# LPMP/BDD

Hardware: AMD Instinct MI355X
Metric: parallel-MMA iterations/sec, 10.5M BDD nodes, 1 GPU (+ achieved HBM GB/s in roofline) (higher is better)
Workload: dtype f32

## Files before the change

bdd_amd/capi.py:

```python
from __future__ import annotations

import ctypes as C
import os
import subprocess

_HERE = os.path.dirname(os.path.abspath(__file__))
LIB_PATH = os.path.abspath(os.environ["BDDMMA_LIB"]) if os.environ.get("BDDMMA_LIB") else os.path.join(_HERE, "csrc", "libbdd_mma_hip.so")

OK = 0
ERR_INVALID_ARGUMENT, ERR_INVALID_BDD, ERR_DEVICE, ERR_STATE, ERR_UNSUPPORTED, ERR_IO = -1, -2, -3, -4, -5, -6
F32, F64 = 0, 1
K_FORWARD_MM, K_BACKWARD_MM, K_FINISH_DELTA, K_OTHER, K_COUNT = 0, 1, 2, 3, 4


class Options(C.Structure):
    _fields_ = [("pack_width", C.c_uint32), ("wide_pack_width", C.c_uint32), ("deterministic", C.c_uint32),
                ("vars_per_bin", C.c_uint32), ("stage_cap", C.c_uint32), ("waves_per_block", C.c_uint32),
                ("keep_bdd_order", C.c_uint32), ("resident_sweeps", C.c_uint32), ("exchange_by_variable", C.c_uint32),
                ("variant_flags", C.c_uint32), ("pack_fill", C.c_uint32), ("pack_stagger", C.c_uint32)]


class LbfgsParams(C.Structure):
    _fields_ = [("history_size", C.c_int32), ("init_step_size", C.c_double), ("req_rel_lb_increase", C.c_double),
                ("step_size_decrease_factor", C.c_double), ("step_size_increase_factor", C.c_double)]
# ... 26 lines not shown
    "bddmma_nr_variables": (_U64, [_V]),
    "bddmma_nr_bdds": (_U64, [_V]),
    "bddmma_nr_layers": (_U64, [_V]),
    "bddmma_nr_bdd_nodes": (_U64, [_V]),
    "bddmma_nr_hops": (_U64, [_V]),
    "bddmma_nr_packs": (_U64, [_V]),
    "bddmma_solve_sweep_kind": (_I, [_V]),
    "bddmma_fused_small": (_I, [_V]),
    "bddmma_fused_small_learned": (_I, [_V]),
    "bddmma_fused_small_history": (_I, [_V]),
    "bddmma_fused_small_stop": (_I, [_V]),
    "bddmma_nontemporal_loads": (_I, [_V]),
    "bddmma_potentials_on_chip": (_I, [_V]),
    "bddmma_onchip_hops": (_I, [_V]),
    "bddmma_lane_sweeps": (_I, [_V]),
    "bddmma_precision": (_I, [_V]),
    "bddmma_device": (_I, [_V]),
    "bddmma_num_bdds_per_var": (_I, [_V, _V]),
    "bddmma_layer_variables": (_I, [_V, _V]),
    "bddmma_layer_bdds": (_I, [_V, _V]),
    "bddmma_nodes_per_hop": (_I, [_V, _V]),
    "bddmma_layers_per_hop": (_I, [_V, _V]),
    "bddmma_update_costs": (_I, [_V, _V, _U64, _V, _U64, _I, _I]),
    "bddmma_set_cost": (_I, [_V, _D, _U64]),
    "bddmma_get_solver_costs": (_I, [_V, _V, _V, _V, _I]),
    "bddmma_set_solver_costs": (_I, [_V, _V, _V, _V, _I]),
    "bddmma_primal_objective_vec": (_I, [_V, _V, _I]),
    "bddmma_forward_run": (_I, [_V]),
    "bddmma_backward_run": (_I, [_V]),
    "bddmma_lower_bound": (_I, [_V, C.POINTER(_D)]),
# ... 71 lines not shown
    "bddmma_set_profiling": (_I, [_V, _I]),
    "bddmma_get_profile": (_I, [_V, C.POINTER(Profile)]),
    "bddmma_time_iterations": (_I, [_V, _D, _U64, C.POINTER(_D)]),
    "bddmma_time_kernel": (_I, [_V, _I, _U64, C.POINTER(_D)]),
    "bddmma_device_bytes": (_U64, [_V]),
    "bddmma_device_allocated_bytes": (_U64, [_V]),
    "bddmma_layout_create": (_I, [C.POINTER(_V), _V, _V, _U64, C.POINTER(Options)]),
    "bddmma_layout_create_for_chip": (_I, [C.POINTER(_V), _V, _V, _U64, C.POINTER(Options), _I, C.c_uint32, C.c_uint32]),
    "bddmma_layout_destroy": (None, [_V]),
    "bddmma_layout_size": (_U64, [_V, _I]),
    "bddmma_layout_copy": (_I, [_V, _I, _V]),
    "bddmma_layout_res2_records": (_I, [_V, _I, _V, _V, _V]),
    "bddmma_layout_stream_records": (_I, [_V, _I, _V, _V, _V]),
    "bddmma_layout_layer_records": (_I, [_V, _I, _V, _V, _V]),
    "bddmma_layout_lane_codes": (_I, [_V, _I, _V, _V, _V]),
    "bddmma_layout_seg_exchange": (_I, [_V, _I, _I, _V, _V, _V, _V]),
}

_I64P, _U64P = C.POINTER(C.c_int64), C.POINTER(C.c_uint64)
ILP_SIGNATURES = {
    "bddilp_last_error": (C.c_char_p, []),
    "bddilp_parse_lp": (_I, [C.c_char_p, C.POINTER(_V)]),
    "bddilp_parse_opb": (_I, [C.c_char_p, C.POINTER(_V)]),
    "bddilp_parse": (_I, [C.c_char_p, C.POINTER(_V)]),
    "bddilp_destroy": (None, [_V]),
    "bddilp_nr_variables": (_U64, [_V]),
    "bddilp_nr_constraints": (_U64, [_V]),
    "bddilp_variable_name": (C.c_char_p, [_V, _U64]),
    "bddilp_objective": (_I, [_V, _V, C.POINTER(_D)]),
    "bddilp_constraint_size": (_U64, [_V, _U64]),
# ... 53 lines not shown
```

bdd_amd/csrc/capi.cpp:

```cpp
#include <chrono>
#include <cmath>
#include <cstdio>
#include <cstdlib>
#include <cstring>
#include <limits>
#include <new>
#include <string>
#include <vector>

#include "../../include/bdd_mma.h"
#include "layout.hpp"
#include "solver.hpp"

using namespace bddmma;

struct bddmma_lbfgs;
extern "C" int bddmma_lbfgs_iteration(bddmma_lbfgs* l);
extern "C" int bddmma_lbfgs_update_costs(bddmma_lbfgs* l, const void* lo, uint64_t n_lo, const void* hi, uint64_t n_hi, int elem_precision,
                                         int on_device);

namespace {
thread_local std::string g_err;

template <typename F>
// ... 122 lines not shown
uint64_t bddmma_nr_variables(const bddmma_solver* s) { return s && s->impl ? s->impl->n_vars : 0; }
uint64_t bddmma_nr_bdds(const bddmma_solver* s) { return s && s->impl ? s->impl->n_bdds : 0; }
uint64_t bddmma_nr_layers(const bddmma_solver* s) { return s && s->impl ? s->impl->n_layers : 0; }
uint64_t bddmma_nr_bdd_nodes(const bddmma_solver* s) { return s && s->impl ? s->impl->n_input_nodes : 0; }
uint64_t bddmma_nr_hops(const bddmma_solver* s) { return s && s->impl ? s->impl->n_hops : 0; }
uint64_t bddmma_nr_packs(const bddmma_solver* s) { return s && s->impl ? s->impl->n_packs_narrow + s->impl->n_packs_wide : 0; }
int bddmma_solve_sweep_kind(const bddmma_solver* s) { return s && s->impl ? s->impl->solve_sweep_kind : -1; }
int bddmma_fused_small(const bddmma_solver* s) { return s && s->impl ? (s->impl->fused_small ? 1 : 0) : -1; }
int bddmma_fused_small_learned(const bddmma_solver* s) { return s && s->impl ? (s->impl->fused_small_learned ? 1 : 0) : -1; }
int bddmma_fused_small_history(const bddmma_solver* s) { return s && s->impl ? (s->impl->fused_small_history ? 1 : 0) : -1; }
int bddmma_fused_small_stop(const bddmma_solver* s) { return s && s->impl ? (s->impl->fused_small_stop ? 1 : 0) : -1; }
int bddmma_nontemporal_loads(const bddmma_solver* s) { return s && s->impl ? (s->impl->nt_loads ? 1 : 0) : -1; }
int bddmma_potentials_on_chip(const bddmma_solver* s) { return s && s->impl ? (s->impl->pot_on_chip ? 1 : 0) : -1; }
int bddmma_onchip_hops(const bddmma_solver* s) { return s && s->impl ? s->impl->onchip_hops : -1; }
int bddmma_lane_sweeps(const bddmma_solver* s) { return s && s->impl ? (s->impl->lane_sweeps ? 1 : 0) : -1; }
int bddmma_precision(const bddmma_solver* s) { return s && s->impl ? s->impl->precision : -1; }
int bddmma_device(const bddmma_solver* s) { return s && s->impl ? s->impl->device : -1; }
uint64_t bddmma_device_bytes(const bddmma_solver* s) { return s && s->impl ? s->impl->dev_bytes : 0; }
uint64_t bddmma_device_allocated_bytes(const bddmma_solver* s) { return s && s->impl ? s->impl->dev_alloc_bytes : 0; }

int bddmma_num_bdds_per_var(const bddmma_solver* s, int32_t* out)
{
    return guarded(s, [&](SolverBase* b) { return copy_host(b->h_nbdds, out); });
}
int bddmma_layer_variables(const bddmma_solver* s, int32_t* out)
{
    return guarded(s, [&](SolverBase* b) { return copy_host(b->h_layer_var, out); });
}
int bddmma_layer_bdds(const bddmma_solver* s, int32_t* out)
{
// ... 799 lines not shown
}

int bddmma_layout_lane_codes(const bddmma_layout* l, int real_size, uint32_t* info, uint32_t* words, uint32_t* code_off)
{
    if (!l || !info || (real_size != 4 && real_size != 8)) return BDDMMA_ERR_INVALID_ARGUMENT;
    LayerRecords R;
    build_layer_records(l->L, (uint32_t)real_size, R);
    LaneCodes K;
    build_lane_codes(l->L, (uint32_t)real_size, R, K);
    info[0] = K.ok ? 1u : 0u; info[1] = (uint32_t)K.words.size(); info[2] = K.affine ? 1u : 0u;
    if (words && !K.words.empty()) std::memcpy(words, K.words.data(), K.words.size() * sizeof(uint32_t));
    if (code_off && !K.code_off.empty()) std::memcpy(code_off, K.code_off.data(), K.code_off.size() * sizeof(uint32_t));
    return BDDMMA_OK;
}

}
```

bdd_amd/csrc/kernels/narrow5.hpp:

```cpp
#pragma once

namespace bddmma {

#ifndef BDDMMA_N5_WAVES
#define BDDMMA_N5_WAVES 5
#endif
constexpr int n5_waves(int hc) { return hc <= 10 ? BDDMMA_N5_WAVES : 4; }

__device__ __forceinline__ uint32_t lane_hop_code(const u4v& cw, int h) { return (cw[h / 3] >> (10 * (h % 3))) & 0x3FFu; }
__device__ __forceinline__ u4v lane_codes_again(const u4v& cw)
{
    uint32_t a = cw[0], b = cw[1], c = cw[2], e = cw[3];
    asm volatile("" : "+v"(a), "+v"(b), "+v"(c), "+v"(e));
    return u4v{a, b, c, e};
}
__device__ __forceinline__ uint32_t lane_bit(uint32_t code, uint32_t bit) { return (uint32_t)__builtin_amdgcn_sbfe((int)code, bit, 1u); }
__device__ __forceinline__ float lane_pick(uint32_t m, float a, float b)
{
    return __builtin_bit_cast(float, (m & __builtin_bit_cast(uint32_t, a)) | (~m & __builtin_bit_cast(uint32_t, b)));
}
__device__ __forceinline__ float lane_child(uint32_t code, uint32_t k, float ta, float tb)
{
    const uint32_t odd = lane_bit(code, k), snk = lane_bit(code, k + 1);
    const float node = lane_pick(odd, tb, ta);
// ... 1 lines not shown
    return lane_pick(snk, sink, node);
}
__device__ __forceinline__ void lane_push(float& fa, float& fb, uint32_t code, float p0, float p1, float p2, float p3)
{
    const float INF = inf_v<float>();
    const float pv[4] = {p0, p1, p2, p3};
    fa = fb = INF;
#pragma unroll
    for (uint32_t k = 0; k < 4; ++k) {
        const uint32_t odd = lane_bit(code, 2 * k), snk = lane_bit(code, 2 * k + 1);
        fa = rmin(fa, lane_pick(odd | snk, INF, pv[k]));
        fb = rmin(fb, lane_pick(odd & ~snk, pv[k], INF));
    }
}

template <typename REAL, int WPB, int HC>
__device__ __forceinline__ void fwd_narrow5_body(const DevPtrs<REAL>& d, const PackDev& pk, const uint32_t* __restrict__ lcode,
                                                 const uint32_t* __restrict__ lcode_off, uint32_t lcode_words, REAL omega, uint32_t block_id)
{
    static_assert(HC + 1 <= (int)HOP_WIN, "one window of hop offsets has to hold the pack");
    static_assert(HC <= (int)LCODE_HOPS, "a lane's code words hold LCODE_HOPS hops");
    using P2 = typename Pair<REAL>::type;
    extern __shared__ __attribute__((aligned(16))) unsigned char dyn_lds[];
    P2* sD = reinterpret_cast<P2*>(dyn_lds);
    __shared__ uint32_t sOffN_[WPB][HOP_WIN], sOffL_[WPB][HOP_WIN], sOffR_[WPB][HOP_WIN];
    const uint32_t tid = threadIdx.x;
    const int wave = __builtin_amdgcn_readfirstlane((int)(tid >> 6));
    const int lane = tid & 63;
    const uint32_t n_quads = (pk.n_packs + WPB - 1) / WPB;
    const uint32_t quad = block_to_pack(block_id, n_quads, pk.xcd_chunk);
    BDDMMA_EXIT_IF(quad >= n_quads, d)
// ... 15 lines not shown
    const REAL* const lohi_p = d.lohi + 2 * (size_t)l0;
    const rsrc_t rc = make_rsrc(lcode, lcode_words);
    HopWindow hw{sOffN_[wave], sOffL_[wave], sOffR_[wave], q0, q1, slot_first, l0};
    uint32_t lb[HC + 1];
    P2 L[HC];
    P2 T[HC + 1];
#pragma unroll
    for (int i = 0; i < HC + 1; ++i) T[i] = P2{REAL(0), REAL(0)};
    const uint32_t db = (uint32_t)wave * pk.stage_cap * (uint32_t)sizeof(P2);
    hw.fill(pk, q0, lane);
#pragma unroll
    for (int i = 0; i < HC + 1; ++i) lb[i] = hw.layer_off(q0 + i);
#pragma unroll
    for (int h = 0; h < HC; ++h)
        hop_load(L[h], rs.lohi, (uint32_t)h < hops ? (uint32_t)lane * (uint32_t)sizeof(P2) : OOB, lb[h] * (uint32_t)sizeof(P2));
    u4v cw = __builtin_amdgcn_raw_buffer_load_b128(rc, (uint32_t)lane * 16u, cbase * 16u, 0);
    {
        REAL ta = REAL(0), tb = REAL(0);
#pragma unroll
        for (int h = HC - 1; h >= 1; --h) {
            if ((uint32_t)h < hops) {
                const uint32_t code = lane_hop_code(cw, h);
                const REAL tla = lane_child(code, 0, ta, tb), tha = lane_child(code, 2, ta, tb);
                const REAL tlb = lane_child(code, 4, ta, tb), thb = lane_child(code, 6, ta, tb);
                const P2 c = L[h];
                ta = rmin(c.y + tha, c.x + tla);
                tb = rmin(c.y + thb, c.x + tlb);
                T[h] = P2{ta, tb};
            }
        }
        BDDMMA_STAMP(p, 5);
    }
    cw = lane_codes_again(cw);
    stage_load_pairs<REAL, WPB>(sD, ent, esl, rs, cnt, tid);
    if (WPB > 1) __syncthreads(); else wave_sync();
    BDDMMA_STAMP(p, 1);
    REAL fa = (lane_hop_code(cw, 0) & (LREC_REAL << 8)) ? REAL(0) : INF, fb = INF;
#pragma unroll
    for (int h = 0; h < HC; ++h) {
        if ((uint32_t)h < hops) {
            const uint32_t code = lane_hop_code(cw, h), flags = code >> 8;
            const uint32_t lbh = lb[h], lbn = lb[h + 1];
            const uint32_t stg = db + (lbh + (uint32_t)lane) * (uint32_t)sizeof(P2);
            const P2 c = L[h];
            const P2 tn = T[h + 1];
            const REAL tla = lane_child(code, 0, tn.x, tn.y), tha = lane_child(code, 2, tn.x, tn.y);
            const REAL tlb = lane_child(code, 4, tn.x, tn.y), thb = lane_child(code, 6, tn.x, tn.y);
            const P2 dd = lds_ld<P2>(dyn_lds, stg);
            const REAL m0 = rmin((fa + c.x) + tla, (fb + c.x) + tlb);
            const REAL m1 = rmin((fa + c.y) + tha, (fb + c.y) + thb);
            const REAL mm = mm_diff1(m0, m1, omega);
            P2 nc;
            nc.x = (c.x + min0(mm)) + dd.x;
            nc.y = (c.y + min0_neg(mm)) + dd.y;
            const rsrc_t rl = hop_rsrc(reinterpret_cast<const P2*>(lohi_p), lbh, lbn - lbh);
            hop_store(nc, rl, (uint32_t)lane * (uint32_t)sizeof(P2), lbh * (uint32_t)sizeof(P2));
            if (flags & LREC_REAL) lds_st<REAL>(dyn_lds, stg, mm);
            const REAL p0 = fa + nc.x, p1 = fa + nc.y, p2 = fb + nc.x, p3 = fb + nc.y;
            lane_push(fa, fb, code, p0, p1, p2, p3);
        }
    }
    BDDMMA_STAMP(p, 3);
    if (WPB > 1) __syncthreads(); else wave_sync();
    BDDMMA_STAMP(p, 2);
    stage_flush<REAL, WPB>(sD, ent, esl, rs, cnt, tid);
    BDDMMA_STAMP(p, 4);
}

template <typename REAL, int WPB, int HC>
__global__ void __launch_bounds__(64 * WPB) __attribute__((amdgpu_waves_per_eu(n5_waves(HC)))) k_fwd_narrow5(DevPtrs<REAL> d, PackDev pk, const uint32_t* __restrict__ lcode, const uint32_t* __restrict__ lcode_off,
                                                          uint32_t lcode_words, REAL omega)
{
    fwd_narrow5_body<REAL, WPB, HC>(d, pk, lcode, lcode_off, lcode_words, omega, blockIdx.x);
}

template <typename REAL, int WPB, int HC>
__device__ __forceinline__ void bwd_narrow5_body(const DevPtrs<REAL>& d, const PackDev& pk, const uint32_t* __restrict__ lcode,
                                                 const uint32_t* __restrict__ lcode_off, uint32_t lcode_words, REAL omega, uint32_t block_id)
{
    static_assert(HC + 1 <= (int)HOP_WIN, "one window of hop offsets has to hold the pack");
    static_assert(HC <= (int)LCODE_HOPS, "a lane's code words hold LCODE_HOPS hops");
    using P2 = typename Pair<REAL>::type;
    extern __shared__ __attribute__((aligned(16))) unsigned char dyn_lds[];
    P2* sD = reinterpret_cast<P2*>(dyn_lds);
    __shared__ uint32_t sOffN_[WPB][HOP_WIN], sOffL_[WPB][HOP_WIN], sOffR_[WPB][HOP_WIN];
    const uint32_t tid = threadIdx.x;
    const int wave = __builtin_amdgcn_readfirstlane((int)(tid >> 6));
    const int lane = tid & 63;
    const uint32_t n_quads = (pk.n_packs + WPB - 1) / WPB;
    const uint32_t quad = block_to_pack(block_id, n_quads, pk.xcd_chunk);
    BDDMMA_EXIT_IF(quad >= n_quads, d)
// ... 15 lines not shown
    const REAL* const lohi_p = d.lohi + 2 * (size_t)l0;
    const rsrc_t rc = make_rsrc(lcode, lcode_words);
    HopWindow hw{sOffN_[wave], sOffL_[wave], sOffR_[wave], q0, q1, slot_first, l0};
    uint32_t lb[HC + 1];
    P2 L[HC];
    P2 F[HC];
#pragma unroll
    for (int i = 0; i < HC; ++i) F[i] = P2{INF, INF};
    const uint32_t db = (uint32_t)wave * pk.stage_cap * (uint32_t)sizeof(P2);
    hw.fill(pk, q0, lane);
#pragma unroll
    for (int i = 0; i < HC + 1; ++i) lb[i] = hw.layer_off(q0 + i);
#pragma unroll
    for (int h = 0; h < HC; ++h)
        hop_load(L[h], rs.lohi, (uint32_t)h < hops ? (uint32_t)lane * (uint32_t)sizeof(P2) : OOB, lb[h] * (uint32_t)sizeof(P2));
    u4v cw = __builtin_amdgcn_raw_buffer_load_b128(rc, (uint32_t)lane * 16u, cbase * 16u, 0);
    {
        REAL fa = (lane_hop_code(cw, 0) & (LREC_REAL << 8)) ? REAL(0) : INF, fb = INF;
#pragma unroll
        for (int h = 0; h < HC; ++h) {
            if ((uint32_t)h < hops) {
                const uint32_t code = lane_hop_code(cw, h);
                if (h >= 1) F[h] = P2{fa, fb};
                if ((uint32_t)h + 1 < hops) {
                    const P2 c = L[h];
                    const REAL p0 = fa + c.x, p1 = fa + c.y, p2 = fb + c.x, p3 = fb + c.y;
                    lane_push(fa, fb, code, p0, p1, p2, p3);
                }
            }
        }
        BDDMMA_STAMP(p, 5);
    }
    cw = lane_codes_again(cw);
    stage_load_pairs<REAL, WPB>(sD, ent, esl, rs, cnt, tid);
    if (WPB > 1) __syncthreads(); else wave_sync();
    BDDMMA_STAMP(p, 1);
    REAL ta = REAL(0), tb = REAL(0);
#pragma unroll
    for (int h = HC - 1; h >= 0; --h) {
        if ((uint32_t)h < hops) {
            const uint32_t code = lane_hop_code(cw, h), flags = code >> 8;
            const uint32_t lbh = lb[h], lbn = lb[h + 1];
            const uint32_t stg = db + (lbh + (uint32_t)lane) * (uint32_t)sizeof(P2);
            const P2 c = L[h];
            const REAL tla = lane_child(code, 0, ta, tb), tha = lane_child(code, 2, ta, tb);
            const REAL tlb = lane_child(code, 4, ta, tb), thb = lane_child(code, 6, ta, tb);
            const P2 dd = lds_ld<P2>(dyn_lds, stg);
            const REAL fa = h >= 1 ? F[h].x : (flags & LREC_REAL) ? REAL(0) : INF;
            const REAL fb = h >= 1 ? F[h].y : INF;
            const REAL m0 = rmin((fa + c.x) + tla, (fb + c.x) + tlb);
            const REAL m1 = rmin((fa + c.y) + tha, (fb + c.y) + thb);
            const REAL mm = mm_diff1(m0, m1, omega);
            P2 nc;
            nc.x = (c.x + min0(mm)) + dd.x;
            nc.y = (c.y + min0_neg(mm)) + dd.y;
            ta = rmin(nc.y + tha, nc.x + tla);
            tb = rmin(nc.y + thb, nc.x + tlb);
            const rsrc_t rl = hop_rsrc(reinterpret_cast<const P2*>(lohi_p), lbh, lbn - lbh);
            hop_store(nc, rl, (uint32_t)lane * (uint32_t)sizeof(P2), lbh * (uint32_t)sizeof(P2));
            if (flags & LREC_REAL) lds_st<REAL>(dyn_lds, stg, mm);
        }
    }
    BDDMMA_STAMP(p, 3);
    if (WPB > 1) __syncthreads(); else wave_sync();
    BDDMMA_STAMP(p, 2);
    stage_flush<REAL, WPB>(sD, ent, esl, rs, cnt, tid);
    BDDMMA_STAMP(p, 4);
    if (!has_pack) return;
    const uint32_t n0 = lb[1] - lb[0];
    double s = 0.0;
    if ((uint32_t)lane < n0) s += (double)ta;
    for (int off2 = 32; off2 > 0; off2 >>= 1) s += __shfl_down(s, off2);
    if (lane == 0) d.lb_partial[pk.lb_base + p] = s;
}

template <typename REAL, int WPB, int HC>
__global__ void __launch_bounds__(64 * WPB) __attribute__((amdgpu_waves_per_eu(n5_waves(HC)))) k_bwd_narrow5(DevPtrs<REAL> d, PackDev pk, const uint32_t* __restrict__ lcode, const uint32_t* __restrict__ lcode_off,
                                                          uint32_t lcode_words, REAL omega)
{
    bwd_narrow5_body<REAL, WPB, HC>(d, pk, lcode, lcode_off, lcode_words, omega, blockIdx.x);
}

}
```

bdd_amd/csrc/layout.cpp:

```cpp
#include "layout.hpp"

#include <algorithm>
#include <atomic>
#include <chrono>
#include <cstdio>
#include <cstdlib>
#include <mutex>
#include <thread>
#include <unordered_map>
#include <cstring>
#include <limits>

namespace bddmma {

namespace {

std::atomic<unsigned> g_layout_threads{0};
thread_local unsigned t_layout_threads = 0;
struct Par {
    unsigned nt = 1;
    Par()
    {
        const char* e = std::getenv("BDDMMA_THREADS");
        const unsigned hw = std::thread::hardware_concurrency();
// ... 1617 lines not shown
                    } else if (off == top) c = LCODE_TOP;
                    else if (off == bot) c = LCODE_BOT;
                    else if (off == na) c = LCODE_A;
                    else if (off == nb) c = LCODE_B;
                    else return;
                    code |= c << (2 * k);
                }
                if (h < LCODE_HOPS) words[(size_t)(first + l) * 4 + h / 3] |= code << (10 * (h % 3));
            }
        }
        for (uint32_t h = nh; h < LCODE_HOPS; ++h)
            for (uint32_t l = 0; l < 64; ++l) words[(size_t)(first + l) * 4 + h / 3] |= 0xFFu << (10 * (h % 3));
    }
    out.affine = true;
    if (!fits || (uint64_t)words.size() * 4 >= (1ull << 31)) return;
    out.words.swap(words);
    out.code_off.swap(code_off);
    out.ok = true;
}

void set_layout_threads(unsigned n) { g_layout_threads.store(n, std::memory_order_relaxed); }
void set_thread_layout_threads(unsigned n) { t_layout_threads = n; }

}
```

bdd_amd/csrc/layout.hpp:

```cpp
#pragma once
#include <cstdint>
#include <string>
#include <vector>

#include "../../include/bdd_mma.h"

#ifndef __host__
#define __host__
#define __device__
#endif

namespace bddmma {

constexpr uint32_t NW_CHILD_BITS = 9;
constexpr uint32_t NW_CHILD_MASK = (1u << NW_CHILD_BITS) - 1;
constexpr uint32_t NW_POS_SHIFT = 18, NW_LIDX_SHIFT = 24, NW_FIELD6 = 63;
constexpr uint32_t NW_TWO = 1u << 30;
constexpr uint32_t NW_PAD = 1u << 31;
constexpr uint32_t nw_top(uint32_t pack_width) { return pack_width; }
constexpr uint32_t nw_bot(uint32_t pack_width) { return pack_width + 1; }
constexpr uint32_t nw_pad_word(uint32_t pack_width)
{
    return NW_PAD | (nw_bot(pack_width) << NW_CHILD_BITS) | nw_bot(pack_width);
}
// ... 168 lines not shown
    std::vector<uint32_t> rec_off;
};
void build_stream_records(const HostLayout& L, uint32_t real_size, StreamRecords& out);

constexpr uint32_t LREC_NO_STORE = 0xFFF0u;
constexpr uint32_t LREC_TWO = 1u, LREC_REAL = 2u;
struct LayerRecords {
    bool ok = false;
    std::vector<uint32_t> rec;
    std::vector<uint32_t> rec_off;
};
void build_layer_records(const HostLayout& L, uint32_t real_size, LayerRecords& out);

constexpr uint32_t LCODE_A = 0u, LCODE_B = 1u, LCODE_TOP = 2u, LCODE_BOT = 3u;
constexpr uint32_t LCODE_HOPS = 12;
struct LaneCodes {
    bool ok = false;
    bool affine = false;
    std::vector<uint32_t> words;
    std::vector<uint32_t> code_off;
};
void build_lane_codes(const HostLayout& L, uint32_t real_size, const LayerRecords& R, LaneCodes& out);

struct LinComb {
    const char* g;
    const void* S;
    const char* Y;
    uint64_t slot;
    const double* cy;
    const double* cs;
    const uint32_t* order;
    int ns;
};
constexpr int LINCOMB_MAX = 8;

// ... 23 lines not shown
```

bdd_amd/csrc/solver.hpp:

```cpp
#pragma once
#include <hip/hip_runtime.h>

#include <cstdint>
#include <limits>
#include <memory>
#include <string>
#include <utility>
#include <vector>

#include "../../include/bdd_mma.h"
#include "layout.hpp"

namespace bddmma {

struct SolverBase {
    int precision = BDDMMA_F32, device = -1;
    hipStream_t stream = nullptr;
    std::string err;
    uint64_t n_vars = 0, n_bdds = 0, n_layers = 0, n_hops = 0, n_input_nodes = 0, n_slots = 0;
    int solve_sweep_kind = 0;
    uint32_t pack_width = 0, wide_pack_width = 0, wide_slot_base = 0;
    uint64_t dev_bytes = 0;
    uint64_t dev_alloc_bytes = 0;
    bool fwd_valid = false, bwd_valid = false;
// ... 35 lines not shown
    }
    virtual int learned_iterations(const void* dist_weights, int weights_on_device, uint64_t num_itr, double omega, double improvement_slope,
                                   void* sol_avg, void* lb_first_diff_avg, void* lb_second_diff_avg, uint64_t compute_history_for_itr,
                                   double history_avg_beta, int outputs_on_device, uint64_t* itr_done, const void* omega_vec,
                                   int omega_vec_on_device) = 0;
    virtual int isotropic_dist_weights(void* out, int on_device) = 0;
    double initial_lb_change = std::numeric_limits<double>::infinity();
    std::shared_ptr<int> lbfgs_attached = std::make_shared<int>(0);
    bool fused_small = false;
    bool fused_small_learned = false;
    bool fused_small_history = false;
    bool fused_small_stop = false;
    bool nt_loads = false;
    bool pot_on_chip = false;
    bool lane_sweeps = false;
    int onchip_hops = 0;
    virtual int run_plain(uint64_t max_iter, double tolerance, double slope, double time_limit, int verbose, bddmma_run_result* res) = 0;
    virtual int forward_mm(double omega, void* delta, int on_device) = 0;
    virtual int backward_mm(double omega, void* delta, int on_device) = 0;
    virtual int normalize_delta(void* delta, int on_device) = 0;
    virtual int distribute_delta() = 0;
    virtual int get_delta(void* out, int on_device) = 0;
    virtual int set_delta(const void* in, int on_device) = 0;
    virtual int update_costs(const void* lo, uint64_t n_lo, const void* hi, uint64_t n_hi, int elem_precision, int on_device) = 0;
    virtual int set_cost(double c, uint64_t var) = 0;
    virtual int get_solver_costs(void* lo, void* hi, void* mm, int on_device) = 0;
    virtual int set_solver_costs(const void* lo, const void* hi, const void* mm, int on_device) = 0;
    virtual int primal_objective_vec(void* out, int on_device) = 0;
    virtual int min_marginals(int sorted, int32_t* var, void* mm0, void* mm1, int on_device) = 0;
    virtual int min_marginal_diff(void* out, int on_device) = 0;
// ... 92 lines not shown
```

bdd_amd/csrc/solver_impl.hpp:

```cpp
#pragma once
#include <hip/hip_runtime.h>
#include <atomic>
#include <chrono>
#include <cmath>
#include <cstdio>
#include <cstdlib>
#include <cstring>
#include <limits>
#include <memory>
#include <string>
#include <thread>
#include <type_traits>
#include <vector>
#include "../../include/bdd_mma.h"
#include "kernels.hpp"
#include "layout.hpp"
#include "solver.hpp"

namespace bddmma {

static inline void cpu_relax()
{
#if defined(__x86_64__) || defined(__i386__)
    __asm__ __volatile__("pause");
// ... 132 lines not shown
    int small_nw = 1;
    uint32_t small_lds = 0;
    SmallDev small{};
    uint32_t* d_small_lds = nullptr;
    bool small_ln_ok = false, small_ln_rl = false, sl_ready = false;
    bool small_stop_ok = false;
    bool small_hist_ok = false;
    uint32_t small_ln_lds = 0;
    SmallDev small_ln{};
    SmallLearn<REAL> small_ln_arg{};
    bool use_narrow3 = false;
    int onchip_hc = 0;
    uint32_t onchip_mode = 0;
    uint32_t *d_lrec = nullptr, *d_lrec_off = nullptr;
    uint32_t lrec_words = 0;
    bool lane5 = false;
    uint32_t *d_lcode = nullptr, *d_lcode_off = nullptr;
    uint32_t lcode_words = 0;
    uint32_t huge_pack_width = 0;
    unsigned char* d_huge_scratch = nullptr;

    std::vector<void*> allocs;

    ~SolverT() override
    {
        if (device >= 0) (void)hipSetDevice(device);
        for (void* p : allocs) (void)hipFree(p);
        if (h_lb) (void)hipHostFree(h_lb);
        if (h_lb_seq) (void)hipHostFree(h_lb_seq);
        if (h_run) (void)hipHostFree(h_run);
        if (d_run_ctl) (void)hipFree(d_run_ctl);
// ... 314 lines not shown
        nt_loads = n3_nt || n12_nt;
        if constexpr (sizeof(REAL) == 4) {
            if (use_narrow3 && res_hdr_ok && !n3_nt && !(opts && (opts->variant_flags & 0x200000u))) {
                uint32_t max_hops = 0;
                for (uint32_t p = 0; p < nb_.n_packs; ++p) max_hops = std::max(max_hops, L.res.pack_hdr[8 * (size_t)p + 5] & 0xFFFFu);
                onchip_hc = max_hops <= 10 ? 10 : max_hops <= 12 ? 12 : max_hops <= 16 ? 16 : 0;
                const uint32_t part = opts ? (opts->variant_flags >> 22) & 3u : 0u;
                if (onchip_hc == 16) onchip_mode = 3;
                if (part == 1 || part == 2) {
                    if (onchip_hc == 10 && wpb == 4) onchip_mode = part;
                    else onchip_hc = 0;
                }
                pot_on_chip = onchip_hc != 0;
                onchip_hops = onchip_hc;
                if ((onchip_hc == 10 || onchip_hc == 12) && onchip_mode == 0 && lane_codes.ok && !(opts && (opts->variant_flags & 0x1000000u))) {
                    if ((rc = upload(&d_lcode, lane_codes.words))) return rc;
                    if ((rc = upload(&d_lcode_off, lane_codes.code_off))) return rc;
                    lcode_words = (uint32_t)lane_codes.words.size();
                    lane5 = lane_sweeps = true;
                }
            }
        }
        if (wb_.n_packs) {
            wide_threads = std::min<uint32_t>(1024, std::max<uint32_t>(64, ((wide_pack_width + 1) / 2 + 63) / 64 * 64));
            wide_npt = (wide_pack_width + wide_threads - 1) / wide_threads;
            wide_npt = wide_npt <= 1 ? 1 : (wide_npt <= 2 ? 2 : 4);
            wide_lds = (uint32_t)wide2_lds_bytes(sizeof(REAL), wide_pack_width, true);
            if (wide_lds > lds_cu || wide_pack_width > 4096) {
                err = "wide_pack_width " + std::to_string(wide_pack_width) + " needs " + std::to_string(wide_lds) + " B of LDS (> 160 KiB)";
                return BDDMMA_ERR_UNSUPPORTED;
            }
        }
        if (wb_.n_packs && nb_.n_packs && !use_res && !(opts && (opts->variant_flags & 1u))) {
            const uint32_t threads = 64 * wpb;
// ... 192 lines not shown
                               return pick<1, 2, 4, 8>(wpb, [&](auto W) {
                                   return pick<1, 2, 4>(mixed_npt, [&](auto N) -> MixedFn {
                                       constexpr int R = PW.value / 64;
                                       return bwd ? &k_bwd_mixed<REAL, R, W.value, N.value, OV> : &k_fwd_mixed<REAL, R, W.value, N.value, OV>;
                                   });
                               });
                           }),
                           mixed_lds};
        }
        return s;
    }
    RecFn onchip_fn(bool bwd, bool rebuild, bool store) const
    {
        if (lane5)
            return pick<4, 8>(wpb, [&](auto W) -> RecFn {
                if (onchip_hc == 12) return bwd ? &k_bwd_narrow5<REAL, W.value, 12> : &k_fwd_narrow5<REAL, W.value, 12>;
                return bwd ? &k_bwd_narrow5<REAL, W.value, 10> : &k_fwd_narrow5<REAL, W.value, 10>;
            });
        if (onchip_hc == 16) return pick<4, 8>(wpb, [&](auto W) -> RecFn { return &k_bwd_narrow4<REAL, W.value, 16, true, true>; });
        if (onchip_hc == 12)
            return pick<4, 8>(wpb, [&](auto W) -> RecFn {
                return bwd ? &k_bwd_narrow4<REAL, W.value, 12, true, false> : &k_fwd_narrow4<REAL, W.value, 12, true, false>;
            });
        if (rebuild && !store)
            return pick<4, 8>(wpb, [&](auto W) -> RecFn {
                return bwd ? &k_bwd_narrow4<REAL, W.value, 10, true, false> : &k_fwd_narrow4<REAL, W.value, 10, true, false>;
            });
        if (rebuild) return bwd ? &k_bwd_narrow4<REAL, 4, 10, true, true> : &k_fwd_narrow4<REAL, 4, 10, true, true>;
        return bwd ? &k_bwd_narrow4<REAL, 4, 10, false, false> : &k_fwd_narrow4<REAL, 4, 10, false, false>;
    }
// ... 1295 lines not shown
```

bdd_amd/solver.py:

```python
from __future__ import annotations

import ctypes as C

import numpy as np

from . import capi
from .bdd_collection import BddCollection


def _ptr(a):
    return a.ctypes.data_as(C.c_void_p) if a is not None else None


def _is_dev(x):
    return hasattr(x, "data_ptr") and bool(getattr(x, "is_cuda", False))


def _dev_ptr(x, n, dtype):
    assert x.is_contiguous() and x.numel() >= n, "device buffer too small or not contiguous"
    assert x.element_size() == np.dtype(dtype).itemsize, "device buffer has the wrong element type"
    return C.c_void_p(x.data_ptr())


class bdd_hip_parallel_mma:
# ... 55 lines not shown
    def fused_small_history(self) -> bool:
        return bool(self._L.bddmma_fused_small_history(self._h))
    def fused_small_stop(self) -> bool:
        return bool(self._L.bddmma_fused_small_stop(self._h))

    def nontemporal_loads(self) -> bool:
        return bool(self._L.bddmma_nontemporal_loads(self._h))

    def potentials_on_chip(self) -> bool:
        return bool(self._L.bddmma_potentials_on_chip(self._h))

    def onchip_hops(self) -> int:
        return int(self._L.bddmma_onchip_hops(self._h))
    def lane_sweeps(self) -> bool:
        return bool(self._L.bddmma_lane_sweeps(self._h))
    def device(self) -> int:
        return int(self._L.bddmma_device(self._h))
    def device_bytes(self): return int(self._L.bddmma_device_bytes(self._h))
    def device_allocated_bytes(self): return int(self._L.bddmma_device_allocated_bytes(self._h))

    def nr_bdds(self, var=None):
        if var is None:
            return int(self._L.bddmma_nr_bdds(self._h))
        return int(self.get_num_bdds_per_var()[var])

    def get_num_bdds_per_var(self):
        out = np.zeros(self.nr_variables(), np.int32)
        self._ck(self._L.bddmma_num_bdds_per_var(self._h, _ptr(out)))
        return out

# ... 797 lines not shown
```

include/bdd_mma.h:

```cpp
#ifndef BDD_MMA_H
#define BDD_MMA_H

#include <stddef.h>
#include <stdint.h>

#ifdef __cplusplus
extern "C" {
#endif

#define BDDMMA_OK 0
#define BDDMMA_ERR_INVALID_ARGUMENT (-1)
#define BDDMMA_ERR_INVALID_BDD (-2)
#define BDDMMA_ERR_DEVICE (-3)
#define BDDMMA_ERR_STATE (-4)
#define BDDMMA_ERR_UNSUPPORTED (-5)
#define BDDMMA_ERR_IO (-6)

#define BDDMMA_F32 0
#define BDDMMA_F64 1

typedef struct bddmma_instruction {
    uint64_t lo;
    uint64_t hi;
    uint64_t index;
// ... 43 lines not shown
    BDDMMA_SWEEPS_STREAMING1 = 2,
    BDDMMA_SWEEPS_STREAMING2 = 3,
    BDDMMA_SWEEPS_STREAMING3 = 4,
    BDDMMA_SWEEPS_RESIDENT1 = 5,
    BDDMMA_SWEEPS_RESIDENT2 = 6
};
int bddmma_solve_sweep_kind(const bddmma_solver* s);
int bddmma_fused_small(const bddmma_solver* s);
int bddmma_fused_small_learned(const bddmma_solver* s);
int bddmma_fused_small_history(const bddmma_solver* s);
int bddmma_fused_small_stop(const bddmma_solver* s);
int bddmma_nontemporal_loads(const bddmma_solver* s);
int bddmma_potentials_on_chip(const bddmma_solver* s);
int bddmma_onchip_hops(const bddmma_solver* s);
int bddmma_lane_sweeps(const bddmma_solver* s);
int bddmma_precision(const bddmma_solver* s);
int bddmma_device(const bddmma_solver* s);
int bddmma_num_bdds_per_var(const bddmma_solver* s, int32_t* out);
int bddmma_layer_variables(const bddmma_solver* s, int32_t* out);
int bddmma_layer_bdds(const bddmma_solver* s, int32_t* out);
int bddmma_nodes_per_hop(const bddmma_solver* s, uint64_t* out);
int bddmma_layers_per_hop(const bddmma_solver* s, uint64_t* out);

int bddmma_update_costs(bddmma_solver* s, const void* lo, uint64_t n_lo, const void* hi, uint64_t n_hi,
                        int elem_precision, int on_device);
int bddmma_set_cost(bddmma_solver* s, double c, uint64_t var);
int bddmma_get_solver_costs(const bddmma_solver* s, void* lo, void* hi, void* deferred_mm_diff, int on_device);
int bddmma_set_solver_costs(bddmma_solver* s, const void* lo, const void* hi, const void* deferred_mm_diff, int on_device);
int bddmma_primal_objective_vec(bddmma_solver* s, void* out, int on_device);

// ... 160 lines not shown
uint64_t bddmma_device_bytes(const bddmma_solver* s);
uint64_t bddmma_device_allocated_bytes(const bddmma_solver* s);

typedef struct bddmma_layout bddmma_layout;
int bddmma_layout_create(bddmma_layout** out, const bddmma_instruction* instr, const uint64_t* bdd_delims,
                         uint64_t n_bdds, const bddmma_options* opts);
int bddmma_layout_create_for_chip(bddmma_layout** out, const bddmma_instruction* instr, const uint64_t* bdd_delims,
                                  uint64_t n_bdds, const bddmma_options* opts, int real_size, uint32_t n_cus, uint32_t lds_bytes_per_cu);
void bddmma_layout_destroy(bddmma_layout* l);
uint64_t bddmma_layout_size(const bddmma_layout* l, int what);
int bddmma_layout_copy(const bddmma_layout* l, int which, void* out);
int bddmma_layout_res2_records(const bddmma_layout* l, int real_size, uint32_t* info, uint32_t* words, uint32_t* rec_off);
int bddmma_layout_stream_records(const bddmma_layout* l, int real_size, uint32_t* info, uint32_t* words, uint32_t* rec_off);
int bddmma_layout_layer_records(const bddmma_layout* l, int real_size, uint32_t* info, uint32_t* words, uint32_t* rec_off);
int bddmma_layout_lane_codes(const bddmma_layout* l, int real_size, uint32_t* info, uint32_t* words, uint32_t* code_off);
int bddmma_layout_seg_exchange(const bddmma_layout* l, int threads, int real_size, uint32_t* info, uint32_t* bin, uint16_t* perm, uint32_t* thr);

#ifdef __cplusplus
}
#endif
#endif
```

Before: 9867.

## Encode per-lane hop codes as wave-wide bitmasks selected via inverse ballot

```diff
diff --git a/bdd_amd/capi.py b/bdd_amd/capi.py
--- a/bdd_amd/capi.py
+++ b/bdd_amd/capi.py
@@ -64,6 +64,7 @@
     "bddmma_potentials_on_chip": (_I, [_V]),
     "bddmma_onchip_hops": (_I, [_V]),
     "bddmma_lane_sweeps": (_I, [_V]),
+    "bddmma_lane_mask_sweeps": (_I, [_V]),
     "bddmma_precision": (_I, [_V]),
     "bddmma_device": (_I, [_V]),
     "bddmma_num_bdds_per_var": (_I, [_V, _V]),
@@ -165,6 +166,7 @@
     "bddmma_layout_stream_records": (_I, [_V, _I, _V, _V, _V]),
     "bddmma_layout_layer_records": (_I, [_V, _I, _V, _V, _V]),
     "bddmma_layout_lane_codes": (_I, [_V, _I, _V, _V, _V]),
+    "bddmma_layout_lane_masks": (_I, [_V, _I, _V, _V, _V]),
     "bddmma_layout_seg_exchange": (_I, [_V, _I, _I, _V, _V, _V, _V]),
 }
 
diff --git a/bdd_amd/csrc/capi.cpp b/bdd_amd/csrc/capi.cpp
--- a/bdd_amd/csrc/capi.cpp
+++ b/bdd_amd/csrc/capi.cpp
@@ -160,6 +160,7 @@
 int bddmma_potentials_on_chip(const bddmma_solver* s) { return s && s->impl ? (s->impl->pot_on_chip ? 1 : 0) : -1; }
 int bddmma_onchip_hops(const bddmma_solver* s) { return s && s->impl ? s->impl->onchip_hops : -1; }
 int bddmma_lane_sweeps(const bddmma_solver* s) { return s && s->impl ? (s->impl->lane_sweeps ? 1 : 0) : -1; }
+int bddmma_lane_mask_sweeps(const bddmma_solver* s) { return s && s->impl ? (s->impl->lane_mask_sweeps ? 1 : 0) : -1; }
 int bddmma_precision(const bddmma_solver* s) { return s && s->impl ? s->impl->precision : -1; }
 int bddmma_device(const bddmma_solver* s) { return s && s->impl ? s->impl->device : -1; }
 uint64_t bddmma_device_bytes(const bddmma_solver* s) { return s && s->impl ? s->impl->dev_bytes : 0; }
@@ -989,4 +990,17 @@
     return BDDMMA_OK;
 }
 
-}
+int bddmma_layout_lane_masks(const bddmma_layout* l, int real_size, uint32_t* info, uint64_t* masks, uint32_t* mask_off)
+{
+    if (!l || !info || (real_size != 4 && real_size != 8)) return BDDMMA_ERR_INVALID_ARGUMENT;
+    LayerRecords R;
+    build_layer_records(l->L, (uint32_t)real_size, R);
+    LaneCodes K;
+    build_lane_codes(l->L, (uint32_t)real_size, R, K);
+    info[0] = K.ok ? 1u : 0u; info[1] = (uint32_t)K.masks.size(); info[2] = K.affine ? 1u : 0u; info[3] = LMASK_ROW; info[4] = LCODE_HOPS;
+    if (masks && !K.masks.empty()) std::memcpy(masks, K.masks.data(), K.masks.size() * sizeof(uint64_t));
+    if (mask_off && !K.mask_off.empty()) std::memcpy(mask_off, K.mask_off.data(), K.mask_off.size() * sizeof(uint32_t));
+    return BDDMMA_OK;
+}
+
+}
diff --git a/bdd_amd/csrc/kernels/narrow5.hpp b/bdd_amd/csrc/kernels/narrow5.hpp
--- a/bdd_amd/csrc/kernels/narrow5.hpp
+++ b/bdd_amd/csrc/kernels/narrow5.hpp
@@ -39,7 +39,59 @@
     }
 }
 
-template <typename REAL, int WPB, int HC>
+struct HopMasks {
+    uint64_t m[LMASK_ROW];
+};
+__device__ __forceinline__ HopMasks lane_masks(const uint64_t* __restrict__ rows, int h)
+{
+    HopMasks r;
+#pragma unroll
+    for (uint32_t b = 0; b < LMASK_ROW; ++b) r.m[b] = rows[(uint32_t)h * LMASK_ROW + b];
+    return r;
+}
+__device__ __forceinline__ uint32_t scalar_again(uint32_t x)
+{
+    asm volatile("" : "+s"(x));
+    return x;
+}
+__device__ __forceinline__ float mask_pick(uint64_t m, float a, float b) { return __builtin_amdgcn_inverse_ballot_w64(m) ? a : b; }
+
+template <bool MASK>
+__device__ __forceinline__ auto hop_sel(const u4v& cw, const HopMasks* hm, int h)
+{
+    if constexpr (MASK) return hm;
+    else return lane_hop_code(cw, h);
+}
+__device__ __forceinline__ float lane_child(const HopMasks* hm, uint32_t k, float ta, float tb)
+{
+    const uint64_t odd = hm->m[k], snk = hm->m[k + 1];
+    const float node = mask_pick(odd, tb, ta);
+    const float sink = mask_pick(odd, inf_v<float>(), 0.0f);
+    return mask_pick(snk, sink, node);
+}
+__device__ __forceinline__ void lane_push(float& fa, float& fb, const HopMasks* hm, float p0, float p1, float p2, float p3)
+{
+    const float INF = inf_v<float>();
+    const float pv[4] = {p0, p1, p2, p3};
+    fa = fb = INF;
+#pragma unroll
+    for (uint32_t k = 0; k < 4; ++k) {
+        const uint64_t odd = hm->m[2 * k], snk = hm->m[2 * k + 1];
+        fa = rmin(fa, mask_pick(~(odd | snk), pv[k], INF));
+        fb = rmin(fb, mask_pick(odd & ~snk, pv[k], INF));
+    }
+}
+__device__ __forceinline__ bool lane_real(uint32_t code, uint32_t, uint32_t) { return (code >> 8) & LREC_REAL; }
+__device__ __forceinline__ bool lane_real(const HopMasks*, uint32_t lane, uint32_t layers) { return lane < layers; }
+
+template <bool MASK>
+__device__ __forceinline__ bool lane_root(const u4v& cw, int lane, uint32_t layers0)
+{
+    if constexpr (MASK) return (uint32_t)lane < layers0;
+    else return lane_hop_code(cw, 0) & (LREC_REAL << 8);
+}
+
+template <typename REAL, int WPB, int HC, bool MASK>
 __device__ __forceinline__ void fwd_narrow5_body(const DevPtrs<REAL>& d, const PackDev& pk, const uint32_t* __restrict__ lcode,
                                                  const uint32_t* __restrict__ lcode_off, uint32_t lcode_words, REAL omega, uint32_t block_id)
 {
@@ -85,15 +137,20 @@
 #pragma unroll
     for (int h = 0; h < HC; ++h)
         hop_load(L[h], rs.lohi, (uint32_t)h < hops ? (uint32_t)lane * (uint32_t)sizeof(P2) : OOB, lb[h] * (uint32_t)sizeof(P2));
-    u4v cw = __builtin_amdgcn_raw_buffer_load_b128(rc, (uint32_t)lane * 16u, cbase * 16u, 0);
+    u4v cw{};
+    if constexpr (!MASK) cw = __builtin_amdgcn_raw_buffer_load_b128(rc, (uint32_t)lane * 16u, cbase * 16u, 0);
+    const uint64_t* const mrows = reinterpret_cast<const uint64_t*>(lcode) + (size_t)cbase * LMASK_ROW;
+    HopMasks hm{};
+    const uint32_t hops_w = MASK ? scalar_again(hops) : hops;
     {
         REAL ta = REAL(0), tb = REAL(0);
 #pragma unroll
         for (int h = HC - 1; h >= 1; --h) {
-            if ((uint32_t)h < hops) {
-                const uint32_t code = lane_hop_code(cw, h);
-                const REAL tla = lane_child(code, 0, ta, tb), tha = lane_child(code, 2, ta, tb);
-                const REAL tlb = lane_child(code, 4, ta, tb), thb = lane_child(code, 6, ta, tb);
+            if ((uint32_t)h < hops_w) {
+                if constexpr (MASK) hm = lane_masks(mrows, h);
+                const auto sel = hop_sel<MASK>(cw, &hm, h);
+                const REAL tla = lane_child(sel, 0, ta, tb), tha = lane_child(sel, 2, ta, tb);
+                const REAL tlb = lane_child(sel, 4, ta, tb), thb = lane_child(sel, 6, ta, tb);
                 const P2 c = L[h];
                 ta = rmin(c.y + tha, c.x + tla);
                 tb = rmin(c.y + thb, c.x + tlb);
@@ -102,21 +159,22 @@
         }
         BDDMMA_STAMP(p, 5);
     }
-    cw = lane_codes_again(cw);
+    if constexpr (!MASK) cw = lane_codes_again(cw);
     stage_load_pairs<REAL, WPB>(sD, ent, esl, rs, cnt, tid);
     if (WPB > 1) __syncthreads(); else wave_sync();
     BDDMMA_STAMP(p, 1);
-    REAL fa = (lane_hop_code(cw, 0) & (LREC_REAL << 8)) ? REAL(0) : INF, fb = INF;
+    REAL fa = lane_root<MASK>(cw, lane, lb[1] - lb[0]) ? REAL(0) : INF, fb = INF;
 #pragma unroll
     for (int h = 0; h < HC; ++h) {
-        if ((uint32_t)h < hops) {
-            const uint32_t code = lane_hop_code(cw, h), flags = code >> 8;
+        if ((uint32_t)h < hops_w) {
+            if constexpr (MASK) hm = lane_masks(mrows, h);
+            const auto sel = hop_sel<MASK>(cw, &hm, h);
             const uint32_t lbh = lb[h], lbn = lb[h + 1];
             const uint32_t stg = db + (lbh + (uint32_t)lane) * (uint32_t)sizeof(P2);
             const P2 c = L[h];
             const P2 tn = T[h + 1];
-            const REAL tla = lane_child(code, 0, tn.x, tn.y), tha = lane_child(code, 2, tn.x, tn.y);
-            const REAL tlb = lane_child(code, 4, tn.x, tn.y), thb = lane_child(code, 6, tn.x, tn.y);
+            const REAL tla = lane_child(sel, 0, tn.x, tn.y), tha = lane_child(sel, 2, tn.x, tn.y);
+            const REAL tlb = lane_child(sel, 4, tn.x, tn.y), thb = lane_child(sel, 6, tn.x, tn.y);
             const P2 dd = lds_ld<P2>(dyn_lds, stg);
             const REAL m0 = rmin((fa + c.x) + tla, (fb + c.x) + tlb);
             const REAL m1 = rmin((fa + c.y) + tha, (fb + c.y) + thb);
@@ -126,9 +184,9 @@
             nc.y = (c.y + min0_neg(mm)) + dd.y;
             const rsrc_t rl = hop_rsrc(reinterpret_cast<const P2*>(lohi_p), lbh, lbn - lbh);
             hop_store(nc, rl, (uint32_t)lane * (uint32_t)sizeof(P2), lbh * (uint32_t)sizeof(P2));
-            if (flags & LREC_REAL) lds_st<REAL>(dyn_lds, stg, mm);
+            if (lane_real(sel, (uint32_t)lane, lbn - lbh)) lds_st<REAL>(dyn_lds, stg, mm);
             const REAL p0 = fa + nc.x, p1 = fa + nc.y, p2 = fb + nc.x, p3 = fb + nc.y;
-            lane_push(fa, fb, code, p0, p1, p2, p3);
+            lane_push(fa, fb, sel, p0, p1, p2, p3);
         }
     }
     BDDMMA_STAMP(p, 3);
@@ -138,14 +196,14 @@
     BDDMMA_STAMP(p, 4);
 }
 
-template <typename REAL, int WPB, int HC>
+template <typename REAL, int WPB, int HC, bool MASK = false>
 __global__ void __launch_bounds__(64 * WPB) __attribute__((amdgpu_waves_per_eu(n5_waves(HC)))) k_fwd_narrow5(DevPtrs<REAL> d, PackDev pk, const uint32_t* __restrict__ lcode, const uint32_t* __restrict__ lcode_off,
                                                           uint32_t lcode_words, REAL omega)
 {
-    fwd_narrow5_body<REAL, WPB, HC>(d, pk, lcode, lcode_off, lcode_words, omega, blockIdx.x);
-}
-
-template <typename REAL, int WPB, int HC>
+    fwd_narrow5_body<REAL, WPB, HC, MASK>(d, pk, lcode, lcode_off, lcode_words, omega, blockIdx.x);
+}
+
+template <typename REAL, int WPB, int HC, bool MASK>
 __device__ __forceinline__ void bwd_narrow5_body(const DevPtrs<REAL>& d, const PackDev& pk, const uint32_t* __restrict__ lcode,
                                                  const uint32_t* __restrict__ lcode_off, uint32_t lcode_words, REAL omega, uint32_t block_id)
 {
@@ -191,39 +249,45 @@
 #pragma unroll
     for (int h = 0; h < HC; ++h)
         hop_load(L[h], rs.lohi, (uint32_t)h < hops ? (uint32_t)lane * (uint32_t)sizeof(P2) : OOB, lb[h] * (uint32_t)sizeof(P2));
-    u4v cw = __builtin_amdgcn_raw_buffer_load_b128(rc, (uint32_t)lane * 16u, cbase * 16u, 0);
+    u4v cw{};
+    if constexpr (!MASK) cw = __builtin_amdgcn_raw_buffer_load_b128(rc, (uint32_t)lane * 16u, cbase * 16u, 0);
+    const uint64_t* const mrows = reinterpret_cast<const uint64_t*>(lcode) + (size_t)cbase * LMASK_ROW;
+    HopMasks hm{};
+    const uint32_t hops_w = MASK ? scalar_again(hops) : hops;
     {
-        REAL fa = (lane_hop_code(cw, 0) & (LREC_REAL << 8)) ? REAL(0) : INF, fb = INF;
+        REAL fa = lane_root<MASK>(cw, lane, lb[1] - lb[0]) ? REAL(0) : INF, fb = INF;
 #pragma unroll
         for (int h = 0; h < HC; ++h) {
-            if ((uint32_t)h < hops) {
-                const uint32_t code = lane_hop_code(cw, h);
+            if ((uint32_t)h < hops_w) {
+                const auto sel = hop_sel<MASK>(cw, &hm, h);
                 if (h >= 1) F[h] = P2{fa, fb};
-                if ((uint32_t)h + 1 < hops) {
+                if ((uint32_t)h + 1 < hops_w) {
+                    if constexpr (MASK) hm = lane_masks(mrows, h);
                     const P2 c = L[h];
                     const REAL p0 = fa + c.x, p1 = fa + c.y, p2 = fb + c.x, p3 = fb + c.y;
-                    lane_push(fa, fb, code, p0, p1, p2, p3);
+                    lane_push(fa, fb, sel, p0, p1, p2, p3);
                 }
             }
         }
         BDDMMA_STAMP(p, 5);
     }
-    cw = lane_codes_again(cw);
+    if constexpr (!MASK) cw = lane_codes_again(cw);
     stage_load_pairs<REAL, WPB>(sD, ent, esl, rs, cnt, tid);
     if (WPB > 1) __syncthreads(); else wave_sync();
     BDDMMA_STAMP(p, 1);
     REAL ta = REAL(0), tb = REAL(0);
 #pragma unroll
     for (int h = HC - 1; h >= 0; --h) {
-        if ((uint32_t)h < hops) {
-            const uint32_t code = lane_hop_code(cw, h), flags = code >> 8;
+        if ((uint32_t)h < hops_w) {
+            if constexpr (MASK) hm = lane_masks(mrows, h);
+            const auto sel = hop_sel<MASK>(cw, &hm, h);
             const uint32_t lbh = lb[h], lbn = lb[h + 1];
             const uint32_t stg = db + (lbh + (uint32_t)lane) * (uint32_t)sizeof(P2);
             const P2 c = L[h];
-            const REAL tla = lane_child(code, 0, ta, tb), tha = lane_child(code, 2, ta, tb);
-            const REAL tlb = lane_child(code, 4, ta, tb), thb = lane_child(code, 6, ta, tb);
+            const REAL tla = lane_child(sel, 0, ta, tb), tha = lane_child(sel, 2, ta, tb);
+            const REAL tlb = lane_child(sel, 4, ta, tb), thb = lane_child(sel, 6, ta, tb);
             const P2 dd = lds_ld<P2>(dyn_lds, stg);
-            const REAL fa = h >= 1 ? F[h].x : (flags & LREC_REAL) ? REAL(0) : INF;
+            const REAL fa = h >= 1 ? F[h].x : lane_real(sel, (uint32_t)lane, lbn - lbh) ? REAL(0) : INF;
             const REAL fb = h >= 1 ? F[h].y : INF;
             const REAL m0 = rmin((fa + c.x) + tla, (fb + c.x) + tlb);
             const REAL m1 = rmin((fa + c.y) + tha, (fb + c.y) + thb);
@@ -235,7 +299,7 @@
             tb = rmin(nc.y + thb, nc.x + tlb);
             const rsrc_t rl = hop_rsrc(reinterpret_cast<const P2*>(lohi_p), lbh, lbn - lbh);
             hop_store(nc, rl, (uint32_t)lane * (uint32_t)sizeof(P2), lbh * (uint32_t)sizeof(P2));
-            if (flags & LREC_REAL) lds_st<REAL>(dyn_lds, stg, mm);
+            if (lane_real(sel, (uint32_t)lane, lbn - lbh)) lds_st<REAL>(dyn_lds, stg, mm);
         }
     }
     BDDMMA_STAMP(p, 3);
@@ -251,11 +315,11 @@
     if (lane == 0) d.lb_partial[pk.lb_base + p] = s;
 }
 
-template <typename REAL, int WPB, int HC>
+template <typename REAL, int WPB, int HC, bool MASK = false>
 __global__ void __launch_bounds__(64 * WPB) __attribute__((amdgpu_waves_per_eu(n5_waves(HC)))) k_bwd_narrow5(DevPtrs<REAL> d, PackDev pk, const uint32_t* __restrict__ lcode, const uint32_t* __restrict__ lcode_off,
                                                           uint32_t lcode_words, REAL omega)
 {
-    bwd_narrow5_body<REAL, WPB, HC>(d, pk, lcode, lcode_off, lcode_words, omega, blockIdx.x);
-}
-
-}
+    bwd_narrow5_body<REAL, WPB, HC, MASK>(d, pk, lcode, lcode_off, lcode_words, omega, blockIdx.x);
+}
+
+}
diff --git a/bdd_amd/csrc/layout.cpp b/bdd_amd/csrc/layout.cpp
--- a/bdd_amd/csrc/layout.cpp
+++ b/bdd_amd/csrc/layout.cpp
@@ -1655,8 +1655,20 @@
     }
     out.affine = true;
     if (!fits || (uint64_t)words.size() * 4 >= (1ull << 31)) return;
+    const size_t n_templates = words.size() / (64 * 4);
+    std::vector<uint64_t> masks(n_templates * LCODE_HOPS * LMASK_ROW, 0ull);
+    for (size_t t = 0; t < n_templates; ++t)
+        for (uint32_t h = 0; h < LCODE_HOPS; ++h)
+            for (uint32_t l = 0; l < 64; ++l) {
+                const uint32_t code = (words[(t * 64 + l) * 4 + h / 3] >> (10 * (h % 3))) & 0x3FFu;
+                for (uint32_t b = 0; b < LMASK_ROW; ++b) masks[(t * LCODE_HOPS + h) * LMASK_ROW + b] |= (uint64_t)((code >> b) & 1u) << l;
+            }
+    std::vector<uint32_t> mask_off(P);
+    for (uint32_t p = 0; p < P; ++p) mask_off[p] = code_off[p] / 64 * LCODE_HOPS;
     out.words.swap(words);
     out.code_off.swap(code_off);
+    out.masks.swap(masks);
+    out.mask_off.swap(mask_off);
     out.ok = true;
 }
 
diff --git a/bdd_amd/csrc/layout.hpp b/bdd_amd/csrc/layout.hpp
--- a/bdd_amd/csrc/layout.hpp
+++ b/bdd_amd/csrc/layout.hpp
@@ -206,11 +206,14 @@
 
 constexpr uint32_t LCODE_A = 0u, LCODE_B = 1u, LCODE_TOP = 2u, LCODE_BOT = 3u;
 constexpr uint32_t LCODE_HOPS = 12;
+constexpr uint32_t LMASK_ROW = 8;
 struct LaneCodes {
     bool ok = false;
     bool affine = false;
     std::vector<uint32_t> words;
     std::vector<uint32_t> code_off;
+    std::vector<uint64_t> masks;
+    std::vector<uint32_t> mask_off;
 };
 void build_lane_codes(const HostLayout& L, uint32_t real_size, const LayerRecords& R, LaneCodes& out);
 
diff --git a/bdd_amd/csrc/solver.hpp b/bdd_amd/csrc/solver.hpp
--- a/bdd_amd/csrc/solver.hpp
+++ b/bdd_amd/csrc/solver.hpp
@@ -73,6 +73,7 @@
     bool nt_loads = false;
     bool pot_on_chip = false;
     bool lane_sweeps = false;
+    bool lane_mask_sweeps = false;
     int onchip_hops = 0;
     virtual int run_plain(uint64_t max_iter, double tolerance, double slope, double time_limit, int verbose, bddmma_run_result* res) = 0;
     virtual int forward_mm(double omega, void* delta, int on_device) = 0;
diff --git a/bdd_amd/csrc/solver_impl.hpp b/bdd_amd/csrc/solver_impl.hpp
--- a/bdd_amd/csrc/solver_impl.hpp
+++ b/bdd_amd/csrc/solver_impl.hpp
@@ -170,7 +170,7 @@
     uint32_t onchip_mode = 0;
     uint32_t *d_lrec = nullptr, *d_lrec_off = nullptr;
     uint32_t lrec_words = 0;
-    bool lane5 = false;
+    bool lane5 = false, lane5_masks = false;
     uint32_t *d_lcode = nullptr, *d_lcode_off = nullptr;
     uint32_t lcode_words = 0;
     uint32_t huge_pack_width = 0;
@@ -515,10 +515,20 @@
                 pot_on_chip = onchip_hc != 0;
                 onchip_hops = onchip_hc;
                 if ((onchip_hc == 10 || onchip_hc == 12) && onchip_mode == 0 && lane_codes.ok && !(opts && (opts->variant_flags & 0x1000000u))) {
-                    if ((rc = upload(&d_lcode, lane_codes.words))) return rc;
-                    if ((rc = upload(&d_lcode_off, lane_codes.code_off))) return rc;
-                    lcode_words = (uint32_t)lane_codes.words.size();
+                    lane5_masks = !(opts && (opts->variant_flags & 0x2000000u));
+                    if (lane5_masks) {
+                        std::vector<uint32_t> mw(lane_codes.masks.size() * 2);
+                        std::memcpy(mw.data(), lane_codes.masks.data(), mw.size() * sizeof(uint32_t));
+                        if ((rc = upload(&d_lcode, mw))) return rc;
+                        if ((rc = upload(&d_lcode_off, lane_codes.mask_off))) return rc;
+                        lcode_words = (uint32_t)mw.size();
+                    } else {
+                        if ((rc = upload(&d_lcode, lane_codes.words))) return rc;
+                        if ((rc = upload(&d_lcode_off, lane_codes.code_off))) return rc;
+                        lcode_words = (uint32_t)lane_codes.words.size();
+                    }
                     lane5 = lane_sweeps = true;
+                    lane_mask_sweeps = lane5_masks;
                 }
             }
         }
@@ -741,6 +751,10 @@
     {
         if (lane5)
             return pick<4, 8>(wpb, [&](auto W) -> RecFn {
+                if (lane5_masks) {
+                    if (onchip_hc == 12) return bwd ? &k_bwd_narrow5<REAL, W.value, 12, true> : &k_fwd_narrow5<REAL, W.value, 12, true>;
+                    return bwd ? &k_bwd_narrow5<REAL, W.value, 10, true> : &k_fwd_narrow5<REAL, W.value, 10, true>;
+                }
                 if (onchip_hc == 12) return bwd ? &k_bwd_narrow5<REAL, W.value, 12> : &k_fwd_narrow5<REAL, W.value, 12>;
                 return bwd ? &k_bwd_narrow5<REAL, W.value, 10> : &k_fwd_narrow5<REAL, W.value, 10>;
             });
diff --git a/bdd_amd/solver.py b/bdd_amd/solver.py
--- a/bdd_amd/solver.py
+++ b/bdd_amd/solver.py
@@ -93,6 +93,9 @@
         return int(self._L.bddmma_onchip_hops(self._h))
     def lane_sweeps(self) -> bool:
         return bool(self._L.bddmma_lane_sweeps(self._h))
+
+    def lane_mask_sweeps(self) -> bool:
+        return bool(self._L.bddmma_lane_mask_sweeps(self._h))
     def device(self) -> int:
         return int(self._L.bddmma_device(self._h))
     def device_bytes(self): return int(self._L.bddmma_device_bytes(self._h))
diff --git a/include/bdd_mma.h b/include/bdd_mma.h
--- a/include/bdd_mma.h
+++ b/include/bdd_mma.h
@@ -81,6 +81,7 @@
 int bddmma_potentials_on_chip(const bddmma_solver* s);
 int bddmma_onchip_hops(const bddmma_solver* s);
 int bddmma_lane_sweeps(const bddmma_solver* s);
+int bddmma_lane_mask_sweeps(const bddmma_solver* s);
 int bddmma_precision(const bddmma_solver* s);
 int bddmma_device(const bddmma_solver* s);
 int bddmma_num_bdds_per_var(const bddmma_solver* s, int32_t* out);
@@ -271,6 +272,7 @@
 int bddmma_layout_stream_records(const bddmma_layout* l, int real_size, uint32_t* info, uint32_t* words, uint32_t* rec_off);
 int bddmma_layout_layer_records(const bddmma_layout* l, int real_size, uint32_t* info, uint32_t* words, uint32_t* rec_off);
 int bddmma_layout_lane_codes(const bddmma_layout* l, int real_size, uint32_t* info, uint32_t* words, uint32_t* code_off);
+int bddmma_layout_lane_masks(const bddmma_layout* l, int real_size, uint32_t* info, uint64_t* masks, uint32_t* mask_off);
 int bddmma_layout_seg_exchange(const bddmma_layout* l, int threads, int real_size, uint32_t* info, uint32_t* bin, uint16_t* perm, uint32_t* thr);
 
 #ifdef __cplusplus
```

Measured after the change: 9681. -1.9%, worse.
